# mmbell/Scythe.jl

Measured on AMD Instinct MI355X. Metric: model steps/sec, RLZ 512x256x64 shallow-water, higher is better.
Workload: dtype f64; 1 GPU; RLZ 513x256x64 (rings x azimuth x levels), 6 vars, 7 derivative slots, Oneway_ShallowWater_HeightResolvedBL, uniform ring table kmax<=127, b_zDim 43; num_cells=171, tiles=1, exchange=none, exchange_impl=none, device_busy_before_warmup=500 steps of the timed model, nan=False

## Files before the change

### scythe.jl_amd/csrc/sx_api.cpp

```cpp
#include "sx_internal.hpp"
#include <algorithm>
#include <array>
#include <cmath>
#include <cstdlib>
#include <cstring>
#include <map>
#include <type_traits>

namespace sx {

static thread_local std::string g_err;
static thread_local bool g_err_set = false;

void set_error(const std::string &msg) {
    if (!g_err_set) g_err = msg;
    g_err_set = true;
}
void clear_error() { g_err_set = false; }
static int status() { return g_err_set ? 1 : 0; }
int error_status() { return status(); }

#define HIPOK(x)                                                                          \
    do {                                                                                  \
        hipError_t e_ = (x);                                                              \
// ... 104 lines not shown
    h->pending.clear();
}

static const int DERIV_SLOTS[4][7] = {
    {0, 1, 2, -1, -1, -1, -1},
    {0, 1, 2, -1, -1, 3, 4},
    {0, 1, 2, 3, 4, -1, -1},
    {0, 1, 2, 3, 4, 5, 6},
};

enum { KU = 1, KR = 2, KRR = 4, KL = 8, KLL = 16, KZ = 32, KZZ = 64 };
enum { KRZ = KU | KR | KRR | KZ | KZZ, KRL = KU | KR | KRR | KL | KLL };
enum { KURZ = KU | KR | KZ, KURL = KU | KR | KL };

struct EqSet {
    int id;
    const char *name;
    int geom, min_vars;
    bool reads_H;
    bool needs_ref;
    int semi_xi, semi_w;
    bool diag_w;
    int kinds[8];
};

static const EqSet EQ_SETS[] = {
    {SX_EQ_LINEAR_ADVECTION_1D,  "LinearAdvection1D",                    SX_GEOM_R,   1, 0, 0, 0, 0, 0, {KU | KR | KRR}},
    {SX_EQ_LINEAR_ADVECTION_RZ,  "LinearAdvectionRZ",                    SX_GEOM_RZ,  4, 0, 0, 0, 0, 0, {KRZ, KU, KU, KU}},
    {SX_EQ_LINEAR_ADVECTION_RL,  "LinearAdvectionRL",                    SX_GEOM_RL,  3, 0, 0, 0, 0, 0, {KRL, KU, KU}},
    {SX_EQ_LINEAR_ADVECTION_RLZ, "LinearAdvectionRLZ",                   SX_GEOM_RLZ, 3, 0, 0, 0, 0, 0, {KRL, KU, KU}},
    {SX_EQ_ONEWAY_SW_SLAB,       "Oneway_ShallowWater_Slab",             SX_GEOM_RL,  6, 0, 0, 0, 0, 1, {KURL, KURL, KURL, KRL, KRL, 0}},
    {SX_EQ_TWOWAY_SW_SLAB,       "Twoway_ShallowWater_Slab",             SX_GEOM_RL,  6, 0, 0, 0, 0, 1, {KURL, KURL, KURL, KRL, KRL, 0}},
    {SX_EQ_ONEWAY_SW_HRBL,       "Oneway_ShallowWater_HeightResolvedBL", SX_GEOM_RLZ, 6, 0, 0, 0, 0, 1,
     {KURL, KURL, KURL, KRL | KZ, KRL | KZ, 0}},
    {SX_EQ_LINEAR_ACOUSTIC_RZ,   "LinearAcousticRZ",                     SX_GEOM_RZ,  5, 0, 0, 0, 0, 0, {KRZ, KURZ, KRZ, KRZ, KRZ}},
    {SX_EQ_EULER_TEST,           "Euler_test",                           SX_GEOM_RZ,  5, 0, 1, 0, 0, 0, {KRZ, KURZ, KRZ, KRZ, KRZ}},
    {SX_EQ_LINEAR_SW_1D,         "LinearShallowWater1D",                 SX_GEOM_R,   2, 1, 0, 0, 0, 0, {KU | KR, KU | KR | KRR}},
    {SX_EQ_LINEAR_SW_RL,         "LinearShallowWaterRL",                 SX_GEOM_RL,  3, 1, 0, 0, 0, 0, {KURL, KU | KR | KRR | KLL, KRL}},
    {SX_EQ_RAINFALL_TEST,        "rainfall_test",                        SX_GEOM_RZ,  8, 0, 1, 2, 5, 0,
     {KRZ, KURZ, KRZ, KRZ, KRZ, KRZ, KRZ, KURZ}},
    {SX_EQ_NONE,                 "None",                                 -1,          1, 0, 0, 0, 0, 0, {KU}},
};

static const EqSet *eq_set(int id) {
    for (const EqSet &e : EQ_SETS)
        if (e.id == id) return &e;
    return nullptr;
}

int default_bzdim(int zDim) {
    int b = (int)std::floor((2.0 * zDim - 1.0) / 3.0) + 1;
    return std::min(zDim, b);
}

static inline int64_t ref_index(int zm, int blk, int node, int K2, int nb) { return ((int64_t)zm * K2 + blk) * nb + node; }
static inline int dev_blk(int b) { return b == 0 ? 0 : b + 1; }

enum SwitchKind {
    FLAG,
    FLAG_AS_2,
    INTEGER
};
struct SwitchRow {
    const char *env;
    int Switches::*i;
    int64_t Switches::*l;
    SwitchKind kind;
    SwitchRow(const char *e, int Switches::*m, SwitchKind k) : env(e), i(m), l(nullptr), kind(k) {}
    SwitchRow(const char *e, int64_t Switches::*m) : env(e), i(nullptr), l(m), kind(INTEGER) {}
};
static const SwitchRow SWITCHES[] = {
    {"SX_OVERLAP", &Switches::overlap, INTEGER},
    {"SX_GRAPH", &Switches::use_graph, FLAG},
    {"SX_NODE_MODE", &Switches::node_mode, FLAG},
    {"SX_DEFER_DIAG", &Switches::defer_diag, FLAG},
    {"SX_FFT_REG", &Switches::fft_reg, FLAG},
    {"SX_DFT_MFMA", &Switches::dft_mfma, FLAG},
    {"SX_DFT_HALFWG", &Switches::dft_half_wg, FLAG},
    {"SX_DFT_EIGHTH", &Switches::dft_eighth, FLAG_AS_2},
    {"SX_DFT_MERGE", &Switches::dft_merge, FLAG},
    {"SX_DFT_RLQ", &Switches::rl_quarter, FLAG},
    {"SX_DFT_HALF", &Switches::dft_half, FLAG},
    {"SX_DFT_CLASSES", &Switches::dft_classes, INTEGER},
    {"SX_FUSE_ZINV", &Switches::fuse_zinv, FLAG},
    {"SX_ZINV_CT", &Switches::zinv_ct, INTEGER},
    {"SX_SBW_MFMA", &Switches::sbw_mfma, INTEGER},
    {"SX_SBW_PF", &Switches::sbw_prefetch, FLAG},
    {"SX_SBW_T256", &Switches::sbw_t256, FLAG},
    {"SX_SBW_SEG", &Switches::sbw_seg, INTEGER},
    {"SX_WIDE", &Switches::wide, FLAG},
    {"SX_SOLVE_PCR", &Switches::solve_pcr, INTEGER},
    {"SX_PCR_MAXCOLS", &Switches::pcr_maxcols},
    {"SX_PCR_R", &Switches::pcr_r, INTEGER},
    {"SX_RZ_FUSED", &Switches::rz_fused, FLAG},
    {"SX_RZ_INV", &Switches::rz_inv, FLAG},
    {"SX_SEMI_MFMA", &Switches::semi_mfma, FLAG},
};

Switches read_switches() {
    Switches sw;
    for (const SwitchRow &r : SWITCHES) {
        const char *v = getenv(r.env);
        if (!v) continue;
        if (r.l) sw.*r.l = atoll(v);
        else sw.*r.i = r.kind == INTEGER ? atoi(v) : atoi(v) == 0 ? 0 : r.kind == FLAG_AS_2 ? 2 : 1;
    }
    return sw;
}

}

using namespace sx;

extern "C" {

const char *sx_last_error(void) { return g_err.c_str(); }
int sx_abi_version(void) { return SX_ABI_VERSION; }

int sx_equation_set_id(const char *name) {
    if (name)
        for (const EqSet &e : EQ_SETS)
            if (!std::strcmp(e.name, name)) return e.id;
    return -1;
}

static int tile_sizes(const sx_grid_desc *g, int n, std::vector<int> &cells) {
    const int nc = g->num_cells;
    if (n < 1 || nc < 3 * n) {
        set_error("calcTileSizes: need at least 3 cells per tile");
        return 1;
    }
    const bool has_l = (g->geometry == SX_GEOM_RL || g->geometry == SX_GEOM_RLZ);
    cells.assign(n, 0);
    if (!has_l || g->ring_uniform_L > 0) {
        for (int t = 0; t < n; t++) cells[t] = nc / n + (t < nc % n ? 1 : 0);
        return 0;
    }
    std::vector<double> cum(nc + 1, 0.0);
    for (int c = 0; c < nc; c++) {
        double pts = 0;
        for (int mu = 0; mu < MUBAR; mu++) pts += 4.0 + 4.0 * (c * MUBAR + mu + 1);
        cum[c + 1] = cum[c] + pts;
    }
    int c0 = 0;
    for (int t = 0; t < n; t++) {
        int c1;
        if (t == n - 1) {
            c1 = nc;
        } else {
            const double target = cum[nc] * (t + 1) / n;
            c1 = c0 + 3;
            while (c1 < nc - 3 * (n - 1 - t) && cum[c1] < target) c1++;
            if (c1 > c0 + 3 && (cum[c1] - target) > (target - cum[c1 - 1])) c1--;
        }
        cells[t] = c1 - c0;
        c0 = c1;
    }
    return 0;
}

int sx_calc_tile_sizes(const sx_grid_desc *g, int32_t n, double *out) {
    clear_error();
    if (!g || !out) { set_error("null argument"); return 1; }
    std::vector<int> cells;
    if (tile_sizes(g, n, cells)) return 1;
    const double DX = (g->xmax - g->xmin) / g->num_cells;
    const bool has_l = (g->geometry == SX_GEOM_RL || g->geometry == SX_GEOM_RLZ);
// ... 1150 lines not shown
```

### scythe.jl_amd/csrc/sx_fft.hip

```cpp
#include "sx_internal.hpp"
#include <cstdlib>
#include <cstdio>
#include <vector>

namespace sx {

constexpr int FFT_FZC = 16;
template <int LOGL> struct FftCfg {
    static constexpr int FZC = FFT_FZC, FNP = FZC / 2, LOGZ = 4, SKEW = (LOGL <= 8) ? 2 : 0;
    static constexpr int L4 = (1 << LOGL) / 4;
    static constexpr int LPT = L4 > 64 ? 64 : L4;
    static constexpr int NB = L4 / LPT;
    static constexpr int NK = 2 * NB;
    static constexpr int THREADS = FNP * LPT < 64 ? 64 : FNP * LPT;
    static constexpr size_t LDS = sizeof(double2) * FNP * ((1 << LOGL) + SKEW);
};

#ifdef SX_PHASES
__device__ long long *g_fft_dbg = nullptr;
#define FFT_STAMP(i) do { if (NODE && threadIdx.x == 0 && g_fft_dbg) g_fft_dbg[((int64_t)(blockIdx.z * gridDim.y + blockIdx.y) * gridDim.x + blockIdx.x) * 8 + (i)] = (long long)__builtin_readcyclecounter(); } while (0)
__device__ long long *g_cells_dbg = nullptr;
#define CELLS_PHASES_BEGIN() long long cp_acc_[6] = {0, 0, 0, 0, 0, 0}, cp_rings_ = 0; asm volatile("" ::: "memory"); const long long cp_t0_ = (long long)__builtin_readcyclecounter(); long long cp_last_ = cp_t0_
#define CELLS_STAMP(i) do { asm volatile("" ::: "memory"); const long long n_ = (long long)__builtin_readcyclecounter(); asm volatile("" ::: "memory"); cp_acc_[i] += n_ - cp_last_; cp_last_ = n_; } while (0)
#define CELLS_RING() (cp_rings_++)
// ... 110 lines not shown

template <int BIT>
__device__ __forceinline__ void fft_swap2(double2 &a, double2 &b, int lane) {
    FftQ A = fft_toq(a), B = fft_toq(b);
#pragma unroll
    for (int i = 0; i < 4; i++) {
        if (BIT == 5) {
            const auto r = __builtin_amdgcn_permlane32_swap(A.d[i], B.d[i], false, false);
            A.d[i] = r[0]; B.d[i] = r[1];
        } else if (BIT == 4) {
            const auto r = __builtin_amdgcn_permlane16_swap(A.d[i], B.d[i], false, false);
            A.d[i] = r[0]; B.d[i] = r[1];
        } else if (BIT == 3) {
            const fft_u32 nb = __builtin_amdgcn_update_dpp(B.d[i], A.d[i], 0x128, 0xF, 0x3, false);
            const fft_u32 na = __builtin_amdgcn_update_dpp(A.d[i], B.d[i], 0x128, 0xF, 0xC, false);
            A.d[i] = na; B.d[i] = nb;
        } else if (BIT == 2) {
            const fft_u32 nb = __builtin_amdgcn_update_dpp(B.d[i], A.d[i], 0x104, 0xF, 0x5, false);
            const fft_u32 na = __builtin_amdgcn_update_dpp(A.d[i], B.d[i], 0x114, 0xF, 0xA, false);
            A.d[i] = na; B.d[i] = nb;
        } else {
            constexpr int ctl = BIT == 1 ? 0x4E : 0xB1;
            const fft_u32 pa = __builtin_amdgcn_mov_dpp(A.d[i], ctl, 0xF, 0xF, false);
            const fft_u32 pb = __builtin_amdgcn_mov_dpp(B.d[i], ctl, 0xF, 0xF, false);
            const bool set = (lane >> BIT) & 1;
            const fft_u32 na = set ? pb : A.d[i], nb = set ? B.d[i] : pa;
            A.d[i] = na; B.d[i] = nb;
        }
    }
    a = fft_fromq(A); b = fft_fromq(B);
}
template <int HI>
__device__ __forceinline__ void fft_transpose4(double2 (&v)[4], int lane) {
    fft_swap2<HI>(v[0], v[2], lane); fft_swap2<HI>(v[1], v[3], lane);
    fft_swap2<HI - 1>(v[0], v[1], lane); fft_swap2<HI - 1>(v[2], v[3], lane);
}
template <int SIGN>
__device__ __forceinline__ void fft_bfly_dif(double2 (&v)[4], double2 w1, bool tw) {
    const double2 t0 = cadd(v[0], v[2]), t1 = csub(v[0], v[2]), t2 = cadd(v[1], v[3]), t3 = cmuli(csub(v[1], v[3]), SIGN);
    const double2 y0 = cadd(t0, t2);
    double2 y1 = cadd(t1, t3), y2 = csub(t0, t2), y3 = csub(t1, t3);
    if (tw) {
        const double2 w2 = cmul(w1, w1), w3 = cmul(w2, w1);
        y1 = cmul(y1, w1); y2 = cmul(y2, w2); y3 = cmul(y3, w3);
    }
    v[0] = y0; v[1] = y1; v[2] = y2; v[3] = y3;
}
template <int SIGN>
__device__ __forceinline__ void fft_reg256(double2 (&v)[4], const double2 (&w)[3], int lane) {
    fft_bfly_dif<SIGN>(v, w[0], true);
    fft_transpose4<5>(v, lane);
    fft_bfly_dif<SIGN>(v, w[1], true);
    fft_transpose4<3>(v, lane);
    fft_bfly_dif<SIGN>(v, w[2], true);
    fft_transpose4<1>(v, lane);
    fft_bfly_dif<SIGN>(v, w[0], false);
}
__device__ __forceinline__ int fft_lb(int lane) { return (lane >> 4) + 4 * ((lane >> 2) & 3) + 16 * (lane & 3); }
__device__ __forceinline__ int fft_pad(int l) { return l + (l >> 4); }
__device__ __forceinline__ double2 fft_bpermute(double2 v, int src_lane) {
    const FftQ q = fft_toq(v);
    FftQ r;
#pragma unroll
    for (int i = 0; i < 4; i++) r.d[i] = (fft_u32)__builtin_amdgcn_ds_bpermute(src_lane << 2, (int)q.d[i]);
    return fft_fromq(r);
}

__device__ __forceinline__ double2 ldpair(const double *p) { return *reinterpret_cast<const double2 *>(p); }
__device__ __forceinline__ double2 ldpair(const float *p) { const float2 v = *reinterpret_cast<const float2 *>(p); return make_double2((double)v.x, (double)v.y); }
__device__ __forceinline__ void stpair(double *p, double2 v) { *reinterpret_cast<double2 *>(p) = v; }
__device__ __forceinline__ void stpair(float *p, double2 v) { *reinterpret_cast<float2 *>(p) = make_float2((float)v.x, (float)v.y); }

struct BinPair { double2 k, n; };
__device__ __forceinline__ BinPair packed_bins(double2 aq, double2 bq, int k, int ld) {
    double2 c = aq, e = bq;
    if (ld == 1) { c = make_double2(-k * aq.y, k * aq.x); e = make_double2(-k * bq.y, k * bq.x); }
    else if (ld == 2) { const double qq = -(double)k * k; c.x *= qq; c.y *= qq; e.x *= qq; e.y *= qq; }
    return {make_double2(c.x - e.y, c.y + e.x), make_double2(c.x + e.y, e.x - c.y)};
}

template <int LOGL, bool REG> struct InvCfg {
    static constexpr int SKEW = REG ? (1 << LOGL) / 16 + 2 : FftCfg<LOGL>::SKEW;
    static constexpr int SET = FftCfg<LOGL>::FNP * ((1 << LOGL) + SKEW);
    static constexpr int TW2 = 3 * 64, NTW = REG ? TW2 + (LOGL == 9 ? 4 * 64 : 0) : 0;
    static constexpr size_t LDS = sizeof(double2) * (2 * SET + NTW);
};
typedef double fft_d4 __attribute__((ext_vector_type(4)));
template <int LOGL, class ST, bool NODE, class AT = double, bool FUSE = false, bool REG = false>
__global__ void __launch_bounds__(512, LOGL <= 8 ? 4 : 2)
k_rl_inverse_fft(const AT *__restrict__ Az, Planes<ST> phys, const double *__restrict__ phi,
                 const int *__restrict__ kmaxr, const int64_t *__restrict__ pstart, const double2 *__restrict__ twg,
                 const int64_t *__restrict__ phoff, const double2 *__restrict__ ph, const int *__restrict__ slotmask,
                 int V, int nz, int nsz, int K2, int nrings, int64_t N, int64_t azrow,
                 int s_u, int s_r, int s_rr, int s_l, int s_ll, int s_z, int s_zz,
                 const double *__restrict__ Asrc = nullptr, int64_t Astride = 0, const double *__restrict__ MzT = nullptr, int Zb = 0,
                 int unit0 = 0) {
    constexpr int L = 1 << LOGL, T = FftCfg<LOGL>::LPT, NK = FftCfg<LOGL>::NK;
    constexpr int FZC = FftCfg<LOGL>::FZC, FNP = FftCfg<LOGL>::FNP, LOGZ = FftCfg<LOGL>::LOGZ;
    constexpr int SKEW = InvCfg<LOGL, REG>::SKEW, SET = InvCfg<LOGL, REG>::SET, TW2 = InvCfg<LOGL, REG>::TW2;
    static_assert(!REG || ((LOGL == 8 || LOGL == 9) && !FUSE), "register-resident passes: 256- and 512-point transforms");
    extern __shared__ double2 smf[];
    FFT_STAMP(0);
    int nslot = 0;
    const int ring = blockIdx.y + unit0, z0 = blockIdx.x * FZC;
    int v = 0;
    for (int u = 0; u < V; u++) {
        const int cu = __popc(slotmask[u]);
        int before = 0;
        for (int w = 0; w < V; w++) { const int cw = __popc(slotmask[w]); before += (cw > cu || (cw == cu && w < u)) ? 1 : 0; }
        if (before == (int)blockIdx.z) v = u;
    }
    const int zc = min(FZC, nz - z0);
    const int km = kmaxr[ring];
    const int f = threadIdx.x / T, t = threadIdx.x - f * T;
    const int za = 2 * f, zb = 2 * f + 1;
    const bool active = (f < FNP) && (za < zc);
    const bool hasb = zb < zc;
    int par = 0;
    Twiddles<LOGL> tw;
    bool setup_done = false;
    const int j0 = NODE ? ring : ring / MUBAR;
    const double2 *phr = ph + phoff[ring];
    const int64_t p0 = pstart[ring];
    const int mask = slotmask[v];
    int kq[NK], kcq[NK];
    bool inq[NK];
    double2 phq[NK];
#pragma unroll
    for (int q = 0; q < NK; q++) {
        kq[q] = t + q * T;
        inq[q] = kq[q] <= km;
        kcq[q] = min(kq[q], K2 / 2 - 1);
        phq[q] = make_double2(1.0, 0.0);
    }
    const bool pair_ok = ((nz & 1) == 0);

    for (int grp = 0; grp < 5; grp++) {
        const int sz = grp < 3 ? 0 : grp - 2, d = grp < 3 ? grp : 0;
        if (sz >= nsz) break;
        const int sl0 = grp == 0 ? s_u : grp == 1 ? s_r : grp == 2 ? s_rr : grp == 3 ? s_z : s_zz;
        const int sl1 = grp == 0 ? s_l : -1, sl2 = grp == 0 ? s_ll : -1;
        const bool n0 = sl0 >= 0 && ((mask >> sl0) & 1), n1 = sl1 >= 0 && ((mask >> sl1) & 1), n2 = sl2 >= 0 && ((mask >> sl2) & 1);
        if (!n0 && !n1 && !n2) continue;
        double2 aq[NK], bq[NK];
        if (FUSE) {
            constexpr int KSM = 16, NWV = (FNP * T) / 64 > 0 ? (FNP * T) / 64 : 1;
            constexpr int TPW = ((L / 16 > 0 ? L / 16 : 1) + NWV - 1) / NWV;
            constexpr int SST = 2 * (L + SKEW) * FNP / FZC;
            const int wave = threadIdx.x >> 6, lane = threadIdx.x & 63, n16 = lane & 15, kk4 = lane >> 4;
            double *S = reinterpret_cast<double *>(smf + par * SET);
            const double *arow = Asrc + (int64_t)j0 * Astride + (int64_t)v * Zb * K2;
            const double *mop = MzT + ((int64_t)v * 3 + sz) * Zb * nz + z0 + n16;
            constexpr int KH = 8;
#pragma unroll
            for (int tt = 0; tt < TPW; tt++) {
                const int tile = wave * TPW + tt;
                const int blk = min(tile * 16 + n16, K2 - 1);
                fft_d4 acc = {0.0, 0.0, 0.0, 0.0};
                int64_t oa = (int64_t)kk4 * nz, ob = (int64_t)kk4 * K2 + blk;
                asm volatile("" : "+v"(oa), "+v"(ob));
                const double *pa = mop + oa, *pb = arow + ob;
#pragma unroll
                for (int k0 = 0; k0 < KSM; k0 += KH) {
                    if (4 * k0 >= Zb) break;
                    double am[KH], bm[KH];
#pragma unroll
                    for (int ks = 0; ks < KH; ks++) {
                        const int k = 4 * (k0 + ks) + kk4;
                        am[ks] = k < Zb ? *pa : 0.0;
                        bm[ks] = (k < Zb && tile * 16 < K2) ? *pb : 0.0;
                        pa += 4 * (int64_t)nz; pb += 4 * (int64_t)K2;
                    }
                    if (!setup_done) {
                        asm volatile("" ::: "memory");
                        int tt2 = t;
                        asm volatile("" : "+v"(tt2));
                        tw.template init<+1>(twg, tt2);
                        asm volatile("" ::: "memory");
                        setup_done = true;
                    }
#pragma unroll
                    for (int ks = 0; ks < KH; ks++)
                        if (4 * (k0 + ks) < Zb) acc = __builtin_amdgcn_mfma_f64_16x16x4f64(am[ks], bm[ks], acc, 0, 0, 0);
                }
                if (tile * 16 < K2) {
#pragma unroll
                    for (int r = 0; r < 4; r++) S[(kk4 + 4 * r) * SST + tile * 16 + n16] = acc[r];
                }
            }
            lds_barrier();
#pragma unroll
            for (int q = 0; q < NK; q++) {
                double2 a1 = make_double2(0.0, 0.0), b1 = a1;
                if (active && inq[q]) {
                    a1 = *reinterpret_cast<const double2 *>(S + za * SST + 2 * kcq[q]);
                    if (hasb) b1 = *reinterpret_cast<const double2 *>(S + zb * SST + 2 * kcq[q]);
                }
                if (kq[q] == 0) { a1.y = 0.0; b1.y = 0.0; }
                aq[q] = a1; bq[q] = b1;
            }
            lds_barrier();
        } else
        {
            constexpr int R = NODE ? 1 : 4;
            const double *pf = phi + ((int64_t)d * nrings + ring) * 4;
            const AT *a0 = Az + (int64_t)j0 * azrow + (((int64_t)v * nsz + sz) * nz + (z0 + (active ? za : 0))) * K2;
            const AT *b0 = a0 + ((active && hasb) ? K2 : 0);
#pragma unroll
            for (int q0 = 0; q0 < NK; q0 += 2) {
                double2 x1[R], y1[R], x2[R], y2[R];
#pragma unroll
                for (int r = 0; r < R; r++) {
                    x1[r] = ldpair(a0 + r * azrow + 2 * kcq[q0]);
                    y1[r] = ldpair(b0 + r * azrow + 2 * kcq[q0]);
                    x2[r] = ldpair(a0 + r * azrow + 2 * kcq[q0 + 1]);
                    y2[r] = ldpair(b0 + r * azrow + 2 * kcq[q0 + 1]);
                }
                if (!setup_done) {
                    asm volatile("" ::: "memory");
                    int tt = t;
                    asm volatile("" : "+v"(tt));
                    if (REG) {
                        double2 *wl = smf + 2 * SET;
                        constexpr int S2 = L / 256;
                        wl[tt] = twg[S2 * tt]; wl[64 + tt] = twg[S2 * 4 * (tt & 15)]; wl[128 + tt] = twg[S2 * 16 * (tt & 3)];
                        if (LOGL == 9) {
#pragma unroll
                            for (int q = 0; q < 4; q++) wl[TW2 + 64 * q + tt] = twg[tt + 64 * q];
                        }
                    } else tw.template init<+1>(twg, tt);
                    if (!NODE) {
#pragma unroll
                        for (int q = 0; q < NK; q++) if (inq[q]) phq[q] = phr[tt + q * T];
                    }
                    asm volatile("" ::: "memory");
                    setup_done = true;
                }
                double2 a1 = make_double2(0.0, 0.0), b1 = a1, a2 = a1, b2 = a1;
#pragma unroll
                for (int r = 0; r < R; r++) {
                    const double fr = pf[r];
                    if (inq[q0]) { a1.x += fr * x1[r].x; a1.y += fr * x1[r].y; b1.x += fr * y1[r].x; b1.y += fr * y1[r].y; }
                    if (inq[q0 + 1]) { a2.x += fr * x2[r].x; a2.y += fr * x2[r].y; b2.x += fr * y2[r].x; b2.y += fr * y2[r].y; }
                }
                if (kq[q0] == 0) { a1.y = 0.0; b1.y = 0.0; }
                if (!hasb) { b1 = make_double2(0.0, 0.0); b2 = b1; }
                if (!NODE) { a1 = cmul(a1, phq[q0]); b1 = cmul(b1, phq[q0]); a2 = cmul(a2, phq[q0 + 1]); b2 = cmul(b2, phq[q0 + 1]); }
                aq[q0] = a1; bq[q0] = b1; aq[q0 + 1] = a2; bq[q0 + 1] = b2;
            }
        }
        if (nslot == 0) FFT_STAMP(1);
        for (int ld = 0; ld < 3; ld++) {
            if (!(ld == 0 ? n0 : ld == 1 ? n1 : n2)) continue;
            const int slot = ld == 0 ? sl0 : ld == 1 ? sl1 : sl2;
            double2 *set = smf + par * SET;
            double2 *X = set + f * (L + SKEW);
            par ^= 1;
            if constexpr (REG) {
                double2 wk[NK], mir[NK];
#pragma unroll
                for (int q = 0; q < NK; q++) {
                    const BinPair w = packed_bins(aq[q], bq[q], kq[q], ld);
                    wk[q] = w.k; mir[q] = kq[q] > 0 ? w.n : make_double2(0.0, 0.0);
                }
                const int src = (64 - t) & 63;
                double2 r[NK];
#pragma unroll
                for (int q = 0; q < NK; q++) r[q] = fft_bpermute(mir[q], src);
                const double2 *wl = smf + 2 * SET;
                const double2 wreg[3] = {wl[t], wl[64 + t], wl[128 + t]};
                const int lb = fft_lb(t);
                if constexpr (LOGL == 8) {
                    double2 v[4] = {wk[0], wk[1], t == 0 ? r[0] : r[1], t == 0 ? r[1] : r[0]};
                    fft_reg256<+1>(v, wreg, t);
                    if (nslot == 0) FFT_STAMP(2); else if (nslot == 1) FFT_STAMP(5);
                    if (active) {
#pragma unroll
                        for (int q = 0; q < 4; q++) X[fft_pad(lb + 64 * q)] = v[q];
                    }
                } else {
                    const double2 hi[4] = {t == 0 ? r[0] : r[3], t == 0 ? r[3] : r[2], t == 0 ? r[2] : r[1], t == 0 ? r[1] : r[0]};
                    double2 ev[4], od[4];
#pragma unroll
                    for (int q = 0; q < 4; q++) {
                        ev[q] = cadd(wk[q], hi[q]);
                        od[q] = cmul(csub(wk[q], hi[q]), wl[TW2 + 64 * q + t]);
                    }
                    fft_reg256<+1>(ev, wreg, t);
                    fft_reg256<+1>(od, wreg, t);
                    if (nslot == 0) FFT_STAMP(2); else if (nslot == 1) FFT_STAMP(5);
                    if (active) {
#pragma unroll
                        for (int q = 0; q < 4; q++) {
                            const int l = 2 * (lb + 64 * q);
                            X[fft_pad(l)] = ev[q];
                            X[fft_pad(l + 1)] = od[q];
                        }
                    }
                }
            } else
            if (active) {
#pragma unroll
                for (int q = 0; q < NK; q++) {
                    const int k = kq[q];
                    const BinPair w = packed_bins(aq[q], bq[q], k, ld);
                    X[k] = w.k;
                    if (k > 0) X[L - k] = w.n;
                    else X[L / 2] = make_double2(0.0, 0.0);
                }
            }
            if (!REG) wave_sync();
            if constexpr (!REG) {
                fft_inplace<LOGL, +1>(X, tw, t, active);
                if (nslot == 0) FFT_STAMP(2); else if (nslot == 1) FFT_STAMP(5);
            }
            lds_barrier();
            if (nslot == 0) FFT_STAMP(3);
            const int zp = threadIdx.x & (FNP - 1);
            const double2 *src2 = set + zp * (L + SKEW);
            auto copy_out = [&](auto *out) {
// ... 192 lines not shown
                double2 v4[4];
#pragma unroll
                for (int q = 0; q < 4; q++) v4[q] = X[at(t + 64 * q)];
                wave_sync();
                fft_reg256<-1>(v4, wreg, t);
                const int lb = fft_lb(t);
#pragma unroll
                for (int q = 0; q < 4; q++) X[at(lb + 64 * q)] = v4[q];
                wave_sync();
            } else
                fft_inplace<LOGL, -1>(X, tw, t, active);
            CELLS_STAMP(2);
            if (active) {
                const double w = wq[ring];
                const double wj[4] = {w * phi[(int64_t)ring * 4], w * phi[(int64_t)ring * 4 + 1], w * phi[(int64_t)ring * 4 + 2], w * phi[(int64_t)ring * 4 + 3]};
#pragma unroll
                for (int q = 0; q < NK; q++) {
                    const int k = t + q * T;
                    if (k > km) continue;
                    const double2 wk = X[at(k)], wn = X[at((L - k) & (L - 1))];
                    double2 xa = make_double2(0.5 * (wk.x + wn.x), 0.5 * (wk.y - wn.y));
                    double2 xb2 = make_double2(0.5 * (wk.y + wn.y), -0.5 * (wk.x - wn.x));
                    double x4[4];
                    if (k == 0) {
                        x4[0] = xa.x * inv; x4[1] = 0.0; x4[2] = xb2.x * inv; x4[3] = 0.0;
                    } else {
                        const double2 pw = cconj(phq[q]);
                        xa = cmul(xa, pw);
                        xb2 = cmul(xb2, pw);
                        x4[0] = xa.x * inv; x4[1] = xa.y * inv; x4[2] = xb2.x * inv; x4[3] = xb2.y * inv;
                    }
#pragma unroll
                    for (int j = 0; j < 4; j++)
#pragma unroll
                        for (int e = 0; e < 4; e++) acc[j][q][e] += wj[j] * x4[e];
                }
            }
            CELLS_STAMP(3);
            CELLS_RING();
        }
        store_node(Fn + (int64_t)c * plane + rowoff, 0);
        CELLS_STAMP(4);
#pragma unroll
        for (int q = 0; q < NK; q++)
#pragma unroll
            for (int e = 0; e < 4; e++) {
                acc[0][q][e] = acc[1][q][e]; acc[1][q][e] = acc[2][q][e]; acc[2][q][e] = acc[3][q][e]; acc[3][q][e] = 0.0;
            }
    }
    double *edge = (cb == ncells) ? Fn + (int64_t)ncells * plane : Fe + (int64_t)seg * 3 * plane;
#pragma unroll
    for (int j = 0; j < 3; j++) store_node(edge + (int64_t)j * plane + rowoff, j);
    CELLS_STAMP(4);
    CELLS_PHASES_END();
}

static int ilog2(int n) { int l = 0; while ((1 << l) < n) l++; return l; }

bool fft_path_ok(const sx_handle *h) {
    const int L = h->uniform_L;
    return h->has_l && L >= 16 && L <= 512 && (L & (L - 1)) == 0;
}

bool fft_fused_zinv(const sx_handle *h) {
    return h->sw.fuse_zinv && h->node_mode && h->has_z && h->uniform_L <= 256 && h->Zb <= 64 && h->nz % 16 == 0 && !h->sp32;
}

struct InvTarget {
    double *out;
    const double *phi;
    const int *kmax;
    const int64_t *pstart, *phoff;
    int n_units, n_phi;
    int64_t N;
    int node_mode;
    int unit0 = 0;
};

template <int LOGL, class ST, bool NODE, class AT, bool FUSE = false, bool REG = false>
static void launch_inv_k(sx_handle *h, const int *d_mask, const InvTarget &tg, const double *az, int64_t azrow) {
    const auto kernel = k_rl_inverse_fft<LOGL, ST, NODE, AT, FUSE, REG>;
    constexpr size_t lds = InvCfg<LOGL, REG>::LDS;
    if (lds > 65536) HIPCHK(hipFuncSetAttribute(reinterpret_cast<const void *>(kernel), hipFuncAttributeMaxDynamicSharedMemorySize, (int)lds));
    const dim3 g((h->nz + FFT_FZC - 1) / FFT_FZC, tg.n_units, h->V);
    hipLaunchKernelGGL(kernel, g, dim3(FftCfg<LOGL>::THREADS), lds, h->stream, reinterpret_cast<const AT *>(az),
                       planes_of<ST>(tg.out, h->V, tg.N), tg.phi, tg.kmax, tg.pstart, h->d_tw, tg.phoff, h->d_ph, d_mask, h->V, h->nz,
                       h->nsz, h->K2, tg.n_phi, tg.N, azrow, h->slot[0], h->slot[1], h->slot[2], h->slot[3], h->slot[4], h->slot[5],
                       h->slot[6], FUSE ? h->d_A + (int64_t)h->cell0 * h->C : nullptr, FUSE ? (int64_t)h->C : 0,
                       FUSE ? h->d_MzT : nullptr, FUSE ? h->Zb : 0, tg.unit0);
}

template <int LOGL, class ST, bool NODE, class AT>
static void launch_inv_v(sx_handle *h, const int *d_mask, const InvTarget &tg, const double *az, int64_t azrow) {
    if constexpr (LOGL == 8 || LOGL == 9) { if (h->sw.fft_reg) { launch_inv_k<LOGL, ST, NODE, AT, false, true>(h, d_mask, tg, az, azrow); return; } }
    launch_inv_k<LOGL, ST, NODE, AT>(h, d_mask, tg, az, azrow);
}

template <int LOGL>
static void launch_inv(sx_handle *h, const int *d_mask, const InvTarget &tg, const double *az, int64_t azrow) {
    if (tg.node_mode && fft_fused_zinv(h)) {
        if (LOGL <= 8) { if (h->f32) launch_inv_k<LOGL, float, true, double, true>(h, d_mask, tg, az, azrow); else launch_inv_k<LOGL, double, true, double, true>(h, d_mask, tg, az, azrow); }
    } else if (h->sp32) {
        if (tg.node_mode) launch_inv_v<LOGL, float, true, float>(h, d_mask, tg, az, azrow); else launch_inv_v<LOGL, float, false, float>(h, d_mask, tg, az, azrow);
    } else if (h->f32) {
        if (tg.node_mode) launch_inv_v<LOGL, float, true, double>(h, d_mask, tg, az, azrow); else launch_inv_v<LOGL, float, false, double>(h, d_mask, tg, az, azrow);
    } else {
        if (tg.node_mode) launch_inv_v<LOGL, double, true, double>(h, d_mask, tg, az, azrow); else launch_inv_v<LOGL, double, false, double>(h, d_mask, tg, az, azrow);
    }
}

static void launch_inv_any(sx_handle *h, const int *d_mask, const InvTarget &tg) {
    if (tg.n_units <= 0) return;
    const double *az = h->has_z ? h->d_Az : h->d_A + (int64_t)h->cell0 * h->C;
    const int64_t azrow = h->has_z ? (int64_t)h->V * 3 * h->nz * h->K2 : h->C;
    switch (ilog2(h->uniform_L)) {
        case 4: launch_inv<4>(h, d_mask, tg, az, azrow); break;
        case 5: launch_inv<5>(h, d_mask, tg, az, azrow); break;
        case 6: launch_inv<6>(h, d_mask, tg, az, azrow); break;
        case 7: launch_inv<7>(h, d_mask, tg, az, azrow); break;
        case 8: launch_inv<8>(h, d_mask, tg, az, azrow); break;
        default: launch_inv<9>(h, d_mask, tg, az, azrow); break;
    }
    HIPCHK(hipGetLastError());
}

template <int LOGL>
static void launch_fwd(sx_handle *h, dim3 g) {
    if (h->sp32)
        hipLaunchKernelGGL((k_fl_forward_fft<LOGL, float>), g, dim3(FftCfg<LOGL>::THREADS), FftCfg<LOGL>::LDS, h->stream, h->d_np1 + (int64_t)h->v_lo * h->N,
                           reinterpret_cast<float *>(h->d_Fl) + (int64_t)h->v_lo * h->nz * h->K2,
                           h->d_kmax, h->d_pstart, h->d_tw, h->d_phoff, h->d_ph, h->V, h->nz, h->K2, h->N);
    else
        hipLaunchKernelGGL((k_fl_forward_fft<LOGL, double>), g, dim3(FftCfg<LOGL>::THREADS), FftCfg<LOGL>::LDS, h->stream, h->d_np1 + (int64_t)h->v_lo * h->N,
                           h->d_Fl + (int64_t)h->v_lo * h->nz * h->K2, h->d_kmax,
                           h->d_pstart, h->d_tw, h->d_phoff, h->d_ph, h->V, h->nz, h->K2, h->N);
}

void launch_rl_inverse_fft(sx_handle *h, const int *d_mask, int n_rings) {
    const int id = timer_id(h, "k_rl_inverse");
    timer_begin(h, id);
    InvTarget tg{h->d_phys, h->d_phi, h->d_kmax, h->d_pstart, h->d_phoff, n_rings < 0 ? h->nrings : n_rings, h->nrings, h->N, 0};
    launch_inv_any(h, d_mask, tg);
    timer_end(h);
}

#ifdef SX_PHASES
static long long *g_fft_buf = nullptr, *g_cells_buf = nullptr;
static int64_t g_fft_n = 0, g_cells_n = 0;
static void phases_dump_one(const char *var, const long long *buf, int64_t n) {
    const char *path = getenv(var);
    if (!path || !buf) return;
    std::vector<long long> hst((size_t)n * 8);
    hipDeviceSynchronize();
    hipMemcpy(hst.data(), buf, sizeof(long long) * hst.size(), hipMemcpyDeviceToHost);
    FILE *f = fopen(path, "wb");
    if (f) { fwrite(hst.data(), sizeof(long long), hst.size(), f); fclose(f); }
}
void fft_phases_dump() {
    phases_dump_one("SX_FFT_PHASES_OUT", g_fft_buf, g_fft_n);
    phases_dump_one("SX_CELLS_PHASES_OUT", g_cells_buf, g_cells_n);
}
#endif

void launch_node_fft(sx_handle *h) {
    const int id = timer_id(h, "k_node_fft");
    timer_begin(h, id);
#ifdef SX_PHASES
    if (!g_fft_buf) {
        g_fft_n = (int64_t)((h->nz + FFT_FZC - 1) / FFT_FZC) * h->V * h->nbt;
        hipMalloc(&g_fft_buf, sizeof(long long) * g_fft_n * 8);
        hipMemset(g_fft_buf, 0, sizeof(long long) * g_fft_n * 8);
        hipMemcpyToSymbol(HIP_SYMBOL(g_fft_dbg), &g_fft_buf, sizeof(g_fft_buf));
    }
#endif
    const int j0 = h->R_in / MUBAR;
    InvTarget tg{h->d_G, h->d_nphi, h->d_nkmax, h->d_npstart, h->d_nphoff, h->nbt - j0, h->nbt, h->NG, 1, j0};
    launch_inv_any(h, h->d_mask_node, tg);
    timer_end(h);
}

template <int LOGL, bool REG>
static void launch_fwd_cells_v(sx_handle *h, const CellsPlan &p) {
    const size_t lds = CellsCfg<LOGL, REG>::LDS;
    if (lds > 65536)
        HIPCHK(hipFuncSetAttribute(reinterpret_cast<const void *>(k_fl_forward_cells<LOGL, REG>), hipFuncAttributeMaxDynamicSharedMemorySize, (int)lds));
    dim3 g(h->nz / FFT_FZC, h->v_cnt, p.segs);
#ifdef SX_PHASES
    if (const int64_t n = (int64_t)g.x * g.y * g.z; n > g_cells_n) {
        if (g_cells_buf) { hipDeviceSynchronize(); hipFree(g_cells_buf); }
        g_cells_n = n;
        hipMalloc(&g_cells_buf, sizeof(long long) * g_cells_n * 8);
        hipMemset(g_cells_buf, 0, sizeof(long long) * g_cells_n * 8);
        hipMemcpyToSymbol(HIP_SYMBOL(g_cells_dbg), &g_cells_buf, sizeof(g_cells_buf));
    }
#endif
    const int64_t plane = (int64_t)h->V * h->nz * h->K2, flo = (int64_t)h->v_lo * h->nz * h->K2;
    hipLaunchKernelGGL((k_fl_forward_cells<LOGL, REG>), g, dim3(p.threads), lds, h->stream, h->d_np1 + (int64_t)h->v_lo * h->N, h->d_Fn + flo,
                       h->d_Fn + (int64_t)h->nbt * plane + flo, h->d_kmax, h->d_pstart, h->d_tw, h->d_phoff, h->d_ph, h->d_phi, h->d_wq,
                       h->V, h->nz, h->K2, h->N, h->ncells, p.S);
}

template <int LOGL>
static void launch_fwd_cells(sx_handle *h, const CellsPlan &p) {
    if constexpr (LOGL == 8) { if (h->sw.fft_reg) { launch_fwd_cells_v<LOGL, true>(h, p); return; } }
    launch_fwd_cells_v<LOGL, false>(h, p);
}

void launch_fl_forward_cells(sx_handle *h, const CellsPlan &p) {
    const int id = timer_id(h, "k_fl_forward");
    timer_begin(h, id);
    switch (p.logL) {
        case 4: launch_fwd_cells<4>(h, p); break;
        case 5: launch_fwd_cells<5>(h, p); break;
        case 6: launch_fwd_cells<6>(h, p); break;
        case 7: launch_fwd_cells<7>(h, p); break;
        default: launch_fwd_cells<8>(h, p); break;
    }
    HIPCHK(hipGetLastError());
    timer_end(h);
}

void launch_fl_forward_fft(sx_handle *h) {
    const int id = timer_id(h, "k_fl_forward");
    timer_begin(h, id);
    dim3 g((h->nz + FFT_FZC - 1) / FFT_FZC, h->v_cnt, h->nrings);
    switch (ilog2(h->uniform_L)) {
        case 4: launch_fwd<4>(h, g); break;
        case 5: launch_fwd<5>(h, g); break;
        case 6: launch_fwd<6>(h, g); break;
        case 7: launch_fwd<7>(h, g); break;
        case 8: launch_fwd<8>(h, g); break;
        default: launch_fwd<9>(h, g); break;
    }
    HIPCHK(hipGetLastError());
    timer_end(h);
}

}
```

### scythe.jl_amd/csrc/sx_internal.hpp

```cpp
#pragma once
#include <hip/hip_runtime.h>
#include <algorithm>
#include <array>
#include <cmath>
#include <cstddef>
#include <cstdint>
#include <memory>
#include <string>
#include <utility>
#include <vector>
#include "scythe_hip.h"

#define HIPCHK(x)                                                                                   \
    do {                                                                                            \
        hipError_t e_ = (x);                                                                        \
        if (e_ != hipSuccess) ::sx::set_error(std::string(#x) + ": " + hipGetErrorString(e_) + " (" __FILE__ ":" + std::to_string(__LINE__) + ")"); \
    } while (0)

namespace sx {

void set_error(const std::string &msg);

constexpr int DFT_KMAX_SINGLE = 319;
constexpr int MUBAR = 3;
// ... 116 lines not shown
    ~DevBuf() { release(); }
    operator T *() const { return p; }
    void release() { if (p) hipFree(p); p = nullptr; cap = 0; }
    void swap(DevBuf &o) { std::swap(p, o.p); std::swap(cap, o.cap); }
    bool alloc(size_t n) {
        release();
        if (hipMalloc((void **)&p, n * sizeof(T)) != hipSuccess) { p = nullptr; return false; }
        cap = n;
        return true;
    }
    bool grow(size_t need, const char *who) {
        if (need <= cap || alloc(need + need / 4)) return true;
        set_error(std::string(who) + ": hipMalloc of the scratch failed");
        return false;
    }
    bool upload(const T *v, size_t n, const char *err) {
        if (alloc(std::max<size_t>(n, 1)) && (!n || hipMemcpy(p, v, sizeof(T) * n, hipMemcpyHostToDevice) == hipSuccess)) return true;
        release();
        set_error(err);
        return false;
    }
    bool upload(const std::vector<T> &v, const char *err) { return upload(v.data(), v.size(), err); }
};
struct DiagState {
    double last_bytes = 0;
    virtual ~DiagState() = default;
};
enum { DIAG_EVAL, DIAG_HARM, DIAG_REDUCE, DIAG_SPEC, DIAG_PARCELS, DIAG_ELLIPTIC, DIAG_EXTREMA, DIAG_CROSSINGS, DIAG_DISTRIBUTION, DIAG_VORTEX, DIAG_STATS, DIAG_ANTIDERIVATIVE, DIAG_ISOSURFACE, DIAG_PROJECT, DIAG_REGRID, DIAG_SCAN, DIAG_COUNT };
struct EvalClasses {
    std::vector<EvalVert> vert;
    std::vector<int> vcls;
    DevBuf<int> d_vcls;
    DevBuf<double> d_w3;
};

template <class ST>
struct Planes {
    double *val;
    ST *der;
};
template <class ST>
__host__ __device__ inline Planes<ST> planes_of(double *base, int V, int64_t n) {
    return Planes<ST>{base, reinterpret_cast<ST *>(base + (int64_t)V * n)};
}

struct CellConsts {
    double phiw[3][MUBAR][4];
    double xmin, DX, goff[MUBAR];
    int gcell0;
};

__device__ __forceinline__ double ab_value(int t, double ts, double u, double e, double e1, double e2) {
    if (t == 1) return u + (ts * e);
    if (t == 2) return u + (0.5 * ts) * ((3.0 * e) - e1);
    return u + ((ts / 12.0) * ((23.0 * e) - (16.0 * e1) + (5.0 * e2)));
}

struct ColJob {
    int64_t in_off, out_off, mat_off;
};

struct SemiArgs {
    double *np1;
    const double *In, *I1, *I2;
    const double *MrecT, *MdzT, *WT, *XT;
    int64_t N;
    int nz, t, wi, xi;
    double ts, tau, pxi;
};

struct Switches {
    int overlap = 0;
    int use_graph = 0;
    int node_mode = 1;
    int defer_diag = 0;
    int fft_reg = 1;
    int dft_mfma = 1;
    int dft_half_wg = 1;
    int dft_eighth = 2;
    int dft_merge = 1;
    int rl_quarter = 1;
    int dft_half = 0;
    int dft_classes = 0;
    int fuse_zinv = 0;
    int zinv_ct = 0;
    int sbw_mfma = 1;
    int sbw_prefetch = 0;
    int sbw_t256 = 1;
    int sbw_seg = 0;
    int wide = 1;
    int solve_pcr = -1;
    int64_t pcr_maxcols = 16384;
    int pcr_r = 0;
    int rz_fused = 1;
    int rz_inv = 1;
    int semi_mfma = 1;
};
Switches read_switches();

enum class SbKernel {
    refused,
    sb, sbz, rz_forward, sbw_32, sbw_32_pf, sbw_64, sbw_64_pf, sbw_128, mfma_32, mfma_64, mfma_64_t256, mfma_128,
    mfma_32_f32, mfma_64_f32, mfma_64_t256_f32, mfma_128_f32
};
struct SbPlan {
    SbKernel kernel = SbKernel::refused;
    int threads = 0, bw = 0;
    int groups = 0, nseg = 0, cps = 0, segs = 0;
};
enum class ZinvKernel { none , colmat, mfma_2_1, mfma_4_1, mfma_4_2, mfma_8_1, mfma_8_2, mfma_8_4 };
struct ZinvPlan {
    ZinvKernel kernel = ZinvKernel::none;
    bool f32 = false;
    int CT = 1, grid_x = 0;
};
struct CellsPlan {
    bool on = false;
    int logL = 0, threads = 0;
    int S = 0, segs = 0;
    SbKernel zk = SbKernel::refused;
    int zthreads = 0, bw = 0, nps = 0, zsegs = 0;
};
struct PcrPlan { int R = 1, logR = 0, threads = 64; };
constexpr int PCR_IPT = 4;
SbPlan plan_sb(int geometry, int nz, int Zb, int K2, int v_cnt, int ncells, int sp32, const Switches &sw);
ZinvPlan plan_zinv(int geometry, int nz, int K2, int sp32, const Switches &sw);
CellsPlan plan_fwd_cells(int geometry, int nz, int Zb, int K2, int nvars, int v_cnt, int ncells, int sp32, int uniform_L, const Switches &sw);
PcrPlan plan_pcr(int nblk_max, int b_rDim, int K2, int ngroups, const Switches &sw);
std::string kernel_name(SbKernel k);
std::string kernel_name(const ZinvPlan &p);

struct Timer {
    const char *name;
    double ms = 0.0;
    int64_t calls = 0;
};

struct PendingEvent {
    int timer;
    hipEvent_t a, b;
};

}

struct sx_handle {
    sx::Switches sw;
    int geom = 0, has_l = 0, has_z = 0;
    double xmin = 0, xmax = 0, DX = 0, l_q = 2.0, zmin = 0, zmax = 0;
    int nc = 0, V = 0, D = 0, ncoord = 1, rDim = 0, b_rDim = 0, nz = 1, Zb = 1, nsz = 1;
    int cell0 = 0, ncells = 0, nrings = 0, nbt = 0, tile_num = 0, uniform_L = 0;
    int kDim = 0, K2 = 1, kDim_t = 0, K2t = 1, kmax_max = 0, L_max = 1;
    int K2ref = 1;
    int64_t N = 0, Nh = 0, C = 0, S_patch = 0, S_tile = 0;
    int slot[7] = {-1, -1, -1, -1, -1, -1, -1};
    std::vector<int> hL, hkmax;
    std::vector<double> hoff;
    std::vector<int64_t> hpstart;
    std::vector<int> bcl, bcl0, bcr, bcb, bct;
    double ts = 0;
    int eq = SX_EQ_NONE, semi = 0, w_index = 0, xi_index = 0, col_var = 0;
    double par[SX_NPARAMS] = {};
    int rot = 0;
    hipStream_t stream = nullptr;
    double *d_A = nullptr, *d_Bfull = nullptr, *d_Btile = nullptr, *d_Btile_own = nullptr;
    const double *d_Bsrc = nullptr;
    int64_t *d_rowoff = nullptr, *d_aoff = nullptr, *d_neg1 = nullptr;
    int a2a_n = 0, a2a_me = 0, a2a_g0 = 0, a2a_g1 = 0;
// ... 158 lines not shown
```

Baseline: 1084 steps/s.

## Enable fused z-inverse in node inverse FFT with register path and block placement

Turns on by default the path that fuses the vertical inverse transform (an MFMA matmul against MzT) into the node inverse FFT. The fused path now also runs with the register-resident 256-point FFT. It restructures the MFMA loop to hold all tile accumulators together with a smaller K step, and flattens the grid so consecutive blocks map chunk and ring in groups of eight to improve locality. This removes a separate z-inverse kernel and its intermediate memory round trip, at the cost of more register pressure and a different block order.

Result: faster. 1103 steps/s (median of 6 runs) (+1.7%).

```diff
diff --git a/scythe.jl_amd/csrc/sx_api.cpp b/scythe.jl_amd/csrc/sx_api.cpp
--- a/scythe.jl_amd/csrc/sx_api.cpp
+++ b/scythe.jl_amd/csrc/sx_api.cpp
@@ -210,7 +210,7 @@
     {"SX_DFT_RLQ", &Switches::rl_quarter, FLAG},
     {"SX_DFT_HALF", &Switches::dft_half, FLAG},
     {"SX_DFT_CLASSES", &Switches::dft_classes, INTEGER},
-    {"SX_FUSE_ZINV", &Switches::fuse_zinv, FLAG},
+    {"SX_FUSE_ZINV", &Switches::fuse_zinv, INTEGER},
     {"SX_ZINV_CT", &Switches::zinv_ct, INTEGER},
     {"SX_SBW_MFMA", &Switches::sbw_mfma, INTEGER},
     {"SX_SBW_PF", &Switches::sbw_prefetch, FLAG},
diff --git a/scythe.jl_amd/csrc/sx_fft.hip b/scythe.jl_amd/csrc/sx_fft.hip
--- a/scythe.jl_amd/csrc/sx_fft.hip
+++ b/scythe.jl_amd/csrc/sx_fft.hip
@@ -216,9 +216,16 @@
 template <int LOGL, bool REG> struct InvCfg {
     static constexpr int SKEW = REG ? (1 << LOGL) / 16 + 2 : FftCfg<LOGL>::SKEW;
     static constexpr int SET = FftCfg<LOGL>::FNP * ((1 << LOGL) + SKEW);
+    static constexpr int SST = 2 * ((1 << LOGL) + SKEW) * FftCfg<LOGL>::FNP / FftCfg<LOGL>::FZC;
+    static constexpr int SLAB = FftCfg<LOGL>::FZC * SST;
+    static_assert(SLAB <= 2 * SET && SST >= (1 << LOGL) && SST % 2 == 0, "the slab fits one set, a row holds L doubles in 16-byte pairs");
     static constexpr int TW2 = 3 * 64, NTW = REG ? TW2 + (LOGL == 9 ? 4 * 64 : 0) : 0;
     static constexpr size_t LDS = sizeof(double2) * (2 * SET + NTW);
 };
+__device__ __forceinline__ void fused_unit_of(int id, int nchunk, bool placed, int &chunk, int &unit) {
+    if (placed) { const int r = id >> 3; chunk = r % nchunk; unit = 8 * (r / nchunk) + (id & 7); }
+    else { chunk = id % nchunk; unit = id / nchunk; }
+}
 typedef double fft_d4 __attribute__((ext_vector_type(4)));
 template <int LOGL, class ST, bool NODE, class AT = double, bool FUSE = false, bool REG = false>
 __global__ void __launch_bounds__(512, LOGL <= 8 ? 4 : 2)
@@ -228,15 +235,20 @@
                  int V, int nz, int nsz, int K2, int nrings, int64_t N, int64_t azrow,
                  int s_u, int s_r, int s_rr, int s_l, int s_ll, int s_z, int s_zz,
                  const double *__restrict__ Asrc = nullptr, int64_t Astride = 0, const double *__restrict__ MzT = nullptr, int Zb = 0,
-                 int unit0 = 0) {
+                 int unit0 = 0, int n_units = 0, int placed = 0) {
     constexpr int L = 1 << LOGL, T = FftCfg<LOGL>::LPT, NK = FftCfg<LOGL>::NK;
     constexpr int FZC = FftCfg<LOGL>::FZC, FNP = FftCfg<LOGL>::FNP, LOGZ = FftCfg<LOGL>::LOGZ;
     constexpr int SKEW = InvCfg<LOGL, REG>::SKEW, SET = InvCfg<LOGL, REG>::SET, TW2 = InvCfg<LOGL, REG>::TW2;
-    static_assert(!REG || ((LOGL == 8 || LOGL == 9) && !FUSE), "register-resident passes: 256- and 512-point transforms");
+    static_assert(!REG || LOGL == 8 || (LOGL == 9 && !FUSE), "register-resident passes: 256- and 512-point transforms; fused at 256");
     extern __shared__ double2 smf[];
     FFT_STAMP(0);
     int nslot = 0;
-    const int ring = blockIdx.y + unit0, z0 = blockIdx.x * FZC;
+    int chunk = blockIdx.x, unit = blockIdx.y;
+    if constexpr (FUSE) {
+        fused_unit_of((int)blockIdx.x, (nz + FZC - 1) / FZC, placed != 0, chunk, unit);
+        if (unit >= n_units) return;
+    }
+    const int ring = unit + unit0, z0 = chunk * FZC;
     int v = 0;
     for (int u = 0; u < V; u++) {
         const int cu = __popc(slotmask[u]);
@@ -268,6 +280,26 @@
         phq[q] = make_double2(1.0, 0.0);
     }
     const bool pair_ok = ((nz & 1) == 0);
+    auto setup = [&]() {
+        asm volatile("" ::: "memory");
+        int tt = t;
+        asm volatile("" : "+v"(tt));
+        if (REG) {
+            double2 *wl = smf + 2 * SET;
+            constexpr int S2 = L / 256;
+            wl[tt] = twg[S2 * tt]; wl[64 + tt] = twg[S2 * 4 * (tt & 15)]; wl[128 + tt] = twg[S2 * 16 * (tt & 3)];
+            if (LOGL == 9) {
+#pragma unroll
+                for (int q = 0; q < 4; q++) wl[TW2 + 64 * q + tt] = twg[tt + 64 * q];
+            }
+        } else tw.template init<+1>(twg, tt);
+        if (!NODE) {
+#pragma unroll
+            for (int q = 0; q < NK; q++) if (inq[q]) phq[q] = phr[tt + q * T];
+        }
+        asm volatile("" ::: "memory");
+        setup_done = true;
+    };
 
     for (int grp = 0; grp < 5; grp++) {
         const int sz = grp < 3 ? 0 : grp - 2, d = grp < 3 ? grp : 0;
@@ -280,46 +312,51 @@
         if (FUSE) {
             constexpr int KSM = 16, NWV = (FNP * T) / 64 > 0 ? (FNP * T) / 64 : 1;
             constexpr int TPW = ((L / 16 > 0 ? L / 16 : 1) + NWV - 1) / NWV;
-            constexpr int SST = 2 * (L + SKEW) * FNP / FZC;
+            constexpr int SST = InvCfg<LOGL, REG>::SST;
             const int wave = threadIdx.x >> 6, lane = threadIdx.x & 63, n16 = lane & 15, kk4 = lane >> 4;
             double *S = reinterpret_cast<double *>(smf + par * SET);
             const double *arow = Asrc + (int64_t)j0 * Astride + (int64_t)v * Zb * K2;
             const double *mop = MzT + ((int64_t)v * 3 + sz) * Zb * nz + z0 + n16;
-            constexpr int KH = 8;
+            constexpr int KH = 4;
+            int64_t oa = (int64_t)kk4 * nz;
+            asm volatile("" : "+v"(oa));
+            const double *pa = mop + oa, *pb[TPW];
+            fft_d4 acc[TPW];
+#pragma unroll
+            for (int tt = 0; tt < TPW; tt++) {
+                int64_t ob = (int64_t)kk4 * K2 + min((wave * TPW + tt) * 16 + n16, K2 - 1);
+                asm volatile("" : "+v"(ob));
+                pb[tt] = arow + ob;
+                acc[tt] = fft_d4{0.0, 0.0, 0.0, 0.0};
+            }
+#pragma unroll
+            for (int k0 = 0; k0 < KSM; k0 += KH) {
+                if (4 * k0 >= Zb) break;
+                double am[KH], bm[TPW][KH];
+#pragma unroll
+                for (int ks = 0; ks < KH; ks++) {
+                    const int k = 4 * (k0 + ks) + kk4;
+                    am[ks] = k < Zb ? *pa : 0.0;
+                    pa += 4 * (int64_t)nz;
+#pragma unroll
+                    for (int tt = 0; tt < TPW; tt++) {
+                        bm[tt][ks] = (k < Zb && (wave * TPW + tt) * 16 < K2) ? *pb[tt] : 0.0;
+                        pb[tt] += 4 * (int64_t)K2;
+                    }
+                }
+                if (!setup_done) setup();
+#pragma unroll
+                for (int tt = 0; tt < TPW; tt++)
+#pragma unroll
+                    for (int ks = 0; ks < KH; ks++)
+                        if (4 * (k0 + ks) < Zb) acc[tt] = __builtin_amdgcn_mfma_f64_16x16x4f64(am[ks], bm[tt][ks], acc[tt], 0, 0, 0);
+            }
 #pragma unroll
             for (int tt = 0; tt < TPW; tt++) {
                 const int tile = wave * TPW + tt;
-                const int blk = min(tile * 16 + n16, K2 - 1);
-                fft_d4 acc = {0.0, 0.0, 0.0, 0.0};
-                int64_t oa = (int64_t)kk4 * nz, ob = (int64_t)kk4 * K2 + blk;
-                asm volatile("" : "+v"(oa), "+v"(ob));
-                const double *pa = mop + oa, *pb = arow + ob;
-#pragma unroll
-                for (int k0 = 0; k0 < KSM; k0 += KH) {
-                    if (4 * k0 >= Zb) break;
-                    double am[KH], bm[KH];
-#pragma unroll
-                    for (int ks = 0; ks < KH; ks++) {
-                        const int k = 4 * (k0 + ks) + kk4;
-                        am[ks] = k < Zb ? *pa : 0.0;
-                        bm[ks] = (k < Zb && tile * 16 < K2) ? *pb : 0.0;
-                        pa += 4 * (int64_t)nz; pb += 4 * (int64_t)K2;
-                    }
-                    if (!setup_done) {
-                        asm volatile("" ::: "memory");
-                        int tt2 = t;
-                        asm volatile("" : "+v"(tt2));
-                        tw.template init<+1>(twg, tt2);
-                        asm volatile("" ::: "memory");
-                        setup_done = true;
-                    }
-#pragma unroll
-                    for (int ks = 0; ks < KH; ks++)
-                        if (4 * (k0 + ks) < Zb) acc = __builtin_amdgcn_mfma_f64_16x16x4f64(am[ks], bm[ks], acc, 0, 0, 0);
-                }
                 if (tile * 16 < K2) {
 #pragma unroll
-                    for (int r = 0; r < 4; r++) S[(kk4 + 4 * r) * SST + tile * 16 + n16] = acc[r];
+                    for (int r = 0; r < 4; r++) S[(kk4 + 4 * r) * SST + tile * 16 + n16] = acc[tt][r];
                 }
             }
             lds_barrier();
@@ -350,26 +387,7 @@
                     x2[r] = ldpair(a0 + r * azrow + 2 * kcq[q0 + 1]);
                     y2[r] = ldpair(b0 + r * azrow + 2 * kcq[q0 + 1]);
                 }
-                if (!setup_done) {
-                    asm volatile("" ::: "memory");
-                    int tt = t;
-                    asm volatile("" : "+v"(tt));
-                    if (REG) {
-                        double2 *wl = smf + 2 * SET;
-                        constexpr int S2 = L / 256;
-                        wl[tt] = twg[S2 * tt]; wl[64 + tt] = twg[S2 * 4 * (tt & 15)]; wl[128 + tt] = twg[S2 * 16 * (tt & 3)];
-                        if (LOGL == 9) {
-#pragma unroll
-                            for (int q = 0; q < 4; q++) wl[TW2 + 64 * q + tt] = twg[tt + 64 * q];
-                        }
-                    } else tw.template init<+1>(twg, tt);
-                    if (!NODE) {
-#pragma unroll
-                        for (int q = 0; q < NK; q++) if (inq[q]) phq[q] = phr[tt + q * T];
-                    }
-                    asm volatile("" ::: "memory");
-                    setup_done = true;
-                }
+                if (!setup_done) setup();
                 double2 a1 = make_double2(0.0, 0.0), b1 = a1, a2 = a1, b2 = a1;
 #pragma unroll
                 for (int r = 0; r < R; r++) {
@@ -728,12 +746,13 @@
     const auto kernel = k_rl_inverse_fft<LOGL, ST, NODE, AT, FUSE, REG>;
     constexpr size_t lds = InvCfg<LOGL, REG>::LDS;
     if (lds > 65536) HIPCHK(hipFuncSetAttribute(reinterpret_cast<const void *>(kernel), hipFuncAttributeMaxDynamicSharedMemorySize, (int)lds));
-    const dim3 g((h->nz + FFT_FZC - 1) / FFT_FZC, tg.n_units, h->V);
+    const int nchunk = (h->nz + FFT_FZC - 1) / FFT_FZC;
+    const dim3 g = FUSE ? dim3(nchunk * 8 * ((tg.n_units + 7) / 8), 1, h->V) : dim3(nchunk, tg.n_units, h->V);
     hipLaunchKernelGGL(kernel, g, dim3(FftCfg<LOGL>::THREADS), lds, h->stream, reinterpret_cast<const AT *>(az),
                        planes_of<ST>(tg.out, h->V, tg.N), tg.phi, tg.kmax, tg.pstart, h->d_tw, tg.phoff, h->d_ph, d_mask, h->V, h->nz,
                        h->nsz, h->K2, tg.n_phi, tg.N, azrow, h->slot[0], h->slot[1], h->slot[2], h->slot[3], h->slot[4], h->slot[5],
                        h->slot[6], FUSE ? h->d_A + (int64_t)h->cell0 * h->C : nullptr, FUSE ? (int64_t)h->C : 0,
-                       FUSE ? h->d_MzT : nullptr, FUSE ? h->Zb : 0, tg.unit0);
+                       FUSE ? h->d_MzT : nullptr, FUSE ? h->Zb : 0, tg.unit0, tg.n_units, h->sw.fuse_zinv != 2);
 }
 
 template <int LOGL, class ST, bool NODE, class AT>
@@ -745,7 +764,12 @@
 template <int LOGL>
 static void launch_inv(sx_handle *h, const int *d_mask, const InvTarget &tg, const double *az, int64_t azrow) {
     if (tg.node_mode && fft_fused_zinv(h)) {
-        if (LOGL <= 8) { if (h->f32) launch_inv_k<LOGL, float, true, double, true>(h, d_mask, tg, az, azrow); else launch_inv_k<LOGL, double, true, double, true>(h, d_mask, tg, az, azrow); }
+        if constexpr (LOGL <= 8) {
+            constexpr bool R8 = LOGL == 8;
+            if (R8 && h->sw.fft_reg) { if (h->f32) launch_inv_k<LOGL, float, true, double, true, R8>(h, d_mask, tg, az, azrow); else launch_inv_k<LOGL, double, true, double, true, R8>(h, d_mask, tg, az, azrow); }
+            else if (h->f32) launch_inv_k<LOGL, float, true, double, true>(h, d_mask, tg, az, azrow);
+            else launch_inv_k<LOGL, double, true, double, true>(h, d_mask, tg, az, azrow);
+        }
     } else if (h->sp32) {
         if (tg.node_mode) launch_inv_v<LOGL, float, true, float>(h, d_mask, tg, az, azrow); else launch_inv_v<LOGL, float, false, float>(h, d_mask, tg, az, azrow);
     } else if (h->f32) {
@@ -813,7 +837,7 @@
     timer_begin(h, id);
 #ifdef SX_PHASES
     if (!g_fft_buf) {
-        g_fft_n = (int64_t)((h->nz + FFT_FZC - 1) / FFT_FZC) * h->V * h->nbt;
+        g_fft_n = (int64_t)((h->nz + FFT_FZC - 1) / FFT_FZC) * h->V * 8 * ((h->nbt + 7) / 8);
         hipMalloc(&g_fft_buf, sizeof(long long) * g_fft_n * 8);
         hipMemset(g_fft_buf, 0, sizeof(long long) * g_fft_n * 8);
         hipMemcpyToSymbol(HIP_SYMBOL(g_fft_dbg), &g_fft_buf, sizeof(g_fft_buf));
diff --git a/scythe.jl_amd/csrc/sx_internal.hpp b/scythe.jl_amd/csrc/sx_internal.hpp
--- a/scythe.jl_amd/csrc/sx_internal.hpp
+++ b/scythe.jl_amd/csrc/sx_internal.hpp
@@ -222,7 +222,7 @@
     int rl_quarter = 1;
     int dft_half = 0;
     int dft_classes = 0;
-    int fuse_zinv = 0;
+    int fuse_zinv = 1;
     int zinv_ct = 0;
     int sbw_mfma = 1;
     int sbw_prefetch = 0;
```
